# 4ment/physher

Hardware: AMD Instinct MI355X
Metric: lnL+gradient evals/sec, 1000-taxon GTR+G4 fp64, 1e6 site patterns (higher is better)
Workload: dtype f64

## Files before the change

include/physher_amd.h:

```cpp
#ifndef PHYSHER_AMD_H
#define PHYSHER_AMD_H

#include <stddef.h>
#include <stdint.h>

#ifdef __cplusplus
extern "C" {
#endif

typedef struct phyamd_engine phyamd_engine;

enum {
	PHYAMD_OK = 0,
	PHYAMD_EINVAL = -1,
	PHYAMD_EDEVICE = -2,
	PHYAMD_ENOMEM = -3,
	PHYAMD_EUNSUPPORTED = -4
};

enum { PHYAMD_RESCALE_NEVER = 0, PHYAMD_RESCALE_ALWAYS = 1, PHYAMD_RESCALE_AUTO = 2 };

enum {
	PHYAMD_GRAD_FOLD_ROOT_FREQS = 1,
	PHYAMD_GRAD_COMPAT_SCALED = 2
// ... 99 lines not shown
int phyamd_get_site_lnl_profile(phyamd_engine *e, phyamd_site_lnl_profile *out);
int phyamd_synchronize(phyamd_engine *e);

int phyamd_get_pattern_log_likelihoods(phyamd_engine *e, double *out );
int phyamd_get_partials(phyamd_engine *e, int node, int upper, double *out);
int phyamd_get_node_matrices(phyamd_engine *e, int node, int derivative, double *out );
int phyamd_post_order_parks(int32_t tip_count, const int32_t *left , const int32_t *right, int32_t root, int32_t second_slot,
                            int32_t *out , int32_t capacity);
#define PHYAMD_PRE_ORDER_COLUMNS 30
int phyamd_pre_order_schedule(int32_t tip_count, const int32_t *left , const int32_t *right, int32_t root, int32_t form,
                              int32_t *out , int32_t capacity, int32_t *hbm_slots);
int phyamd_post_order_slots(int32_t tip_count, const int32_t *left , const int32_t *right, int32_t root,
                            int32_t *out , int32_t capacity, int32_t *slots);
int phyamd_stream_elisions(int32_t tip_count, const int32_t *left , const int32_t *right, int32_t root,
                           int32_t *out , int32_t capacity);
int phyamd_is_rescaling(phyamd_engine *e);
int phyamd_set_rescaling(phyamd_engine *e, int policy);
int phyamd_set_keep_partials(phyamd_engine *e, int on);

typedef struct {
	double matrices_ms, lower_ms, upper_ms, reduce_ms;
	int32_t lower_launches, upper_launches;
	int64_t device_bytes;
	int32_t tiles;
} phyamd_profile;
int phyamd_set_reduction_levels(phyamd_engine *e, int levels);
int phyamd_set_profiling(phyamd_engine *e, int on);
int phyamd_get_profile(phyamd_engine *e, phyamd_profile *out);

#ifdef __cplusplus
// ... 4 lines not shown
```

physher_amd/_lib.py:

```python
from __future__ import annotations

import ctypes as C
import os

_HERE = os.path.dirname(os.path.abspath(__file__))
LIB_PATH = os.environ.get("PHYAMD_LIB") or os.path.join(_HERE, "libphysher_amd.so")

ABI_VERSION = 5

OK, EINVAL, EDEVICE, ENOMEM, EUNSUPPORTED = 0, -1, -2, -3, -4
RESCALE_NEVER, RESCALE_ALWAYS, RESCALE_AUTO = 0, 1, 2
GRAD_FOLD_ROOT_FREQS, GRAD_COMPAT_SCALED = 1, 2


class Config(C.Structure):
    _fields_ = [
        ("tip_count", C.c_int32), ("pattern_count", C.c_int32), ("state_count", C.c_int32),
        ("category_count", C.c_int32), ("device", C.c_int32), ("rescale", C.c_int32),
        ("max_device_bytes", C.c_int64), ("stream", C.c_void_p),
    ]


class Profile(C.Structure):
    _fields_ = [
# ... 91 lines not shown
    ("phyamd_branch_hessian", C.c_int, [_P, C.c_int, _P, _P, _P]),
    ("phyamd_get_hessian_profile", C.c_int, [_P, C.POINTER(HessianProfile)]),
    ("phyamd_get_general_profile", C.c_int, [_P, C.POINTER(GeneralProfile)]),
    ("phyamd_gradient_batch_weights", C.c_int, [_P, C.c_int, C.c_int32, _P, _P, _P, _P]),
    ("phyamd_get_weight_batch_profile", C.c_int, [_P, C.POINTER(WeightBatchProfile)]),
    ("phyamd_pattern_log_likelihoods_trees", C.c_int, [_P, C.c_int, C.c_int32, _P, _P, _P, _P, _P, _P, C.c_int32, _P, _P]),
    ("phyamd_get_site_lnl_profile", C.c_int, [_P, C.POINTER(SiteLnlProfile)]),
    ("phyamd_synchronize", C.c_int, [_P]),
    ("phyamd_get_pattern_log_likelihoods", C.c_int, [_P, _P]),
    ("phyamd_get_partials", C.c_int, [_P, C.c_int, C.c_int, _P]),
    ("phyamd_get_node_matrices", C.c_int, [_P, C.c_int, C.c_int, _P]),
    ("phyamd_post_order_parks", C.c_int, [C.c_int32, _P, _P, C.c_int32, C.c_int32, _P, C.c_int32]),
    ("phyamd_post_order_slots", C.c_int, [C.c_int32, _P, _P, C.c_int32, _P, C.c_int32, _P]),
    ("phyamd_pre_order_schedule", C.c_int, [C.c_int32, _P, _P, C.c_int32, C.c_int32, _P, C.c_int32, _P]),
    ("phyamd_stream_elisions", C.c_int, [C.c_int32, _P, _P, C.c_int32, _P, C.c_int32]),
    ("phyamd_is_rescaling", C.c_int, [_P]),
    ("phyamd_set_rescaling", C.c_int, [_P, C.c_int]),
    ("phyamd_set_keep_partials", C.c_int, [_P, C.c_int]),
    ("phyamd_set_reduction_levels", C.c_int, [_P, C.c_int]),
    ("phyamd_set_profiling", C.c_int, [_P, C.c_int]),
    ("phyamd_get_profile", C.c_int, [_P, C.POINTER(Profile)]),
    ("phyamd_store", C.c_int, [_P]),
    ("phyamd_restore", C.c_int, [_P]),
    ("phyamd_compress_patterns", C.c_int, [C.c_int, C.c_int32, C.c_int64, _P, _P, C.POINTER(C.c_int32), _P, _P]),
]

_lib = None


def load():
# ... 21 lines not shown
```

physher_amd/csrc/phyamd_abi.inc:

```

#include <condition_variable>
#include <functional>
#include <mutex>
#include <thread>

namespace {

class ShardWorkers {
public:
	explicit ShardWorkers(int n) : done_(0), generation_(0), stop_(false) {
		for (int i = 0; i < n; i++) threads_.emplace_back([this, i] { loop(i); });
	}
	~ShardWorkers() {
		{
			std::lock_guard<std::mutex> lk(m_);
			stop_ = true;
			generation_++;
		}
		cv_.notify_all();
		for (auto &t : threads_) t.join();
	}
	void run(const std::function<void(int)> &fn) {
		std::unique_lock<std::mutex> lk(m_);
		fn_ = &fn;
// ... 854 lines not shown
	if (!left || !right) return fail(PHYAMD_EINVAL, "null left or right");
	if (capacity < 0 || (capacity > 0 && !out)) return fail(PHYAMD_EINVAL, "null out with capacity %d", capacity);
	Schedule sched;
	StreamTables stream_tab;
	const std::string err = build_schedule(TreeRef{tip_count, left, right, root}, ScheduleOptions{}, &sched);
	if (!err.empty()) return fail(PHYAMD_EINVAL, "%s", err.c_str());
	build_stream_tables(sched, StreamGeometry{1, 1, WAVE, true}, &stream_tab);
	const std::vector<StreamElision> &el = stream_tab.elisions;
	for (int i = 0; i < (int)el.size() && i < capacity; i++) {
		const int32_t rec[8] = {el[i].node, el[i].parent, el[i].stored, el[i].sibling, el[i].sibling_kind, el[i].source, el[i].side, el[i].chunk};
		std::memcpy(out + (size_t)i * 8, rec, sizeof(rec));
	}
	return (int)el.size();
}

int phyamd_is_rescaling(phyamd_engine *g) {
	CHECK_GROUP(g);
	int any = 0;
	for (Shard *s : g->shards) any |= shard_is_rescaling(s);
	return any;
}

int phyamd_get_profile(phyamd_engine *g, phyamd_profile *out) {
	CHECK_GROUP(g);
	if (!out) return fail(PHYAMD_EINVAL, "null out");
	int rc;
	if ((rc = shard_get_profile(g->shards[0], out))) return rc;
	for (int i = 1; i < group_size(g); i++) {
		phyamd_profile p;
		if ((rc = shard_get_profile(g->shards[i], &p))) return rc;
// ... 12 lines not shown
```

physher_amd/csrc/phyamd_launch.inc:

```

size_t gen_image_doubles(const Shard *e) {
	return e->S == 20 ? MatImage<2, 5>::SIZE : e->S == 60 ? MatImage<4, 15>::SIZE : MatImage<4, 16>::SIZE;
}

template <int RT, int KT>
void launch_matrix_images(Shard *e, int count, const double *src, double *dst, const double *rowscale) {
	hipLaunchKernelGGL((k_matrix_images<RT, KT>), dim3(count), dim3(256), 0, e->stream, e->S, src, dst, rowscale);
}

void build_matrix_images(Shard *e, int count, const double *src, double *dst, const double *rowscale = nullptr) {
	if (e->S == 20) launch_matrix_images<2, 5>(e, count, src, dst, rowscale);
	else if (e->S == 60) launch_matrix_images<4, 15>(e, count, src, dst, rowscale);
	else launch_matrix_images<4, 16>(e, count, src, dst, rowscale);
}

int update_matrices(Shard *e) {
	if (e->generic && e->state.qimg_dirty && e->have_Q && e->have_freqs) {
		build_matrix_images(e, 1, e->d_Q, e->d_imgs + (size_t)e->N * e->C * gen_image_doubles(e));
		build_matrix_images(e, 1, e->d_Q, e->d_imgs + ((size_t)e->N * e->C + 1) * gen_image_doubles(e), e->d_freqs);
		HIP_TRY(hipGetLastError());
		q_images_rebuilt(e);
	}
	if (!e->state.matrices_dirty) return PHYAMD_OK;
	if (e->have_eigen) {
// ... 379 lines not shown
int launch_upper_stream(Shard *e) {
	int rc;
	const int nb = (e->P + WAVE - 1) / WAVE, R = e->stream_tab.R, nops = (int)e->stream_tab.ops.size();
	if ((size_t)nb * e->C * R > (size_t)e->N * e->C * e->gpart_row) return fail(PHYAMD_EDEVICE, "gradient slab too small for the streamed walk");
	e->d_gslab = e->d_gpart;
	if (e->stream_tab.P != e->P || e->stream_tab.mstride != e->mstride) {
		if ((rc = upload_schedule(e))) return rc;
		if (e->stream_tab.P != e->P || e->stream_tab.mstride != e->mstride) return fail(PHYAMD_EDEVICE, "streamed walk: descriptors do not match the pattern storage");
	}
	if ((rc = e->d_oct.ensure((size_t)8 * e->C * R))) return rc;
	const StreamVariant v = stream_variant(e->lower_form, SCALE);
	if (v.scale < 0) return fail(PHYAMD_EDEVICE, "streamed walk: the stored lowers hold the %s form, which no %s post-order pass writes", form_name(e->lower_form), SCALE ? "rescaled" : "plain");
	const bool exp2 = v.scale == 2, tf = v.tf;
	if (exp2 && (rc = e->d_uexp.ensure(std::max<size_t>(1, upper_slots_held(e)) * e->C * e->P))) return rc;
	const int waves = SCALE && !exp2 ? e->C : STREAM_WAVES;
	const size_t lds = (size_t)STREAM_LDS_PER_WAVE * waves + (exp2 ? (size_t)waves * STREAM_PARK_SLOTS * WAVE * sizeof(int) : SCALE ? (size_t)4 * e->C * WAVE * sizeof(double) : 0);
	const dim3 grid_x(SCALE && !exp2 ? (unsigned)nb : (unsigned)((nb + STREAM_WAVES - 1) / STREAM_WAVES) * e->C), block(WAVE, waves);
	hipLaunchKernelGGL(k_op_tables, dim3(nops, e->C), dim3(64), 0, e->stream, nops, e->C, (const int *)e->d_stream_op_tips, (const int *)e->d_stream_op_deep,
	                   (const int *)e->d_stream_site_tab, e->d_mats, FOLD ? e->d_Q : e->d_Qpi, reinterpret_cast<double *>(e->d_optab.get()));
	const int subtrees = (int)e->sched.walk_chunk_off.size() - 2;
	for (int phase = 0; phase < (subtrees > 0 ? 2 : 1); phase++) {
		const bool amb = e->stream_ambiguous;
		auto *kernel = exp2 ? (amb ? k_upper4_stream<FOLD, 2, true, true> : k_upper4_stream<FOLD, 2, false, true>)
		             : SCALE ? (amb ? k_upper4_stream<FOLD, 1, true, false> : k_upper4_stream<FOLD, 1, false, false>)
		             : tf    ? (amb ? k_upper4_stream<FOLD, 0, true, true> : k_upper4_stream<FOLD, 0, false, true>)
		                     : (amb ? k_upper4_stream<FOLD, 0, true, false> : k_upper4_stream<FOLD, 0, false, false>);
		const bool plain = !tf && !e->stream_tab.plain_desc.empty();
		hipLaunchKernelGGL(kernel, dim3(grid_x.x, phase ? subtrees : 1), block, lds, e->stream,
		                   (const StreamDesc *)e->d_stream_ops + (plain ? e->stream_tab.desc.size() : 0), (const StreamChunk *)e->d_stream_chunks + (plain ? e->stream_tab.chunks.size() : 0),
		                   (const int *)e->d_walk_chunk_off, phase, nops, e->P, e->C, nb, (const uint32_t *)e->d_mstream, e->mstride, (const double *)e->d_lower, e->d_upper,
		                   (const double *)e->d_mats, (const char *)e->d_optab, (const double *)(FOLD ? e->d_Q : e->d_Qpi), (const double *)e->d_freqs, (const double *)e->d_wl,
// ... 417 lines not shown
```

physher_amd/csrc/phyamd_schedule.inc:

```

int bind_device(Shard *e) {
	HIP_TRY(hipSetDevice(e->device));
	return PHYAMD_OK;
}

size_t node_partial_doubles(const Shard *e) { return (size_t)e->C * e->S * (e->generic ? e->Pp : e->P); }
size_t lower_slots(const Shard *e) { return e->d_lower.size() / node_partial_doubles(e); }
size_t upper_slots_held(const Shard *e) { return e->d_upper.size() / node_partial_doubles(e); }

int ensure_lower_storage(Shard *e) {
	const size_t need = (size_t)std::max(1, e->sched.core_count) * (e->two_slots ? 2 : 1);
	if (lower_slots(e) >= need) return PHYAMD_OK;
	e->d_lower.release();
	e->d_lscale.release();
	return e->d_lower.ensure(need * node_partial_doubles(e));
}

void refresh_op_cores(Schedule &s) {
	for (std::vector<NodeOp> *ops : {&s.lower_ops, &s.upper_ops, &s.walk_lower_ops, &s.walk_upper_ops, &s.walk_chunk_ops, &s.walk_lower_chunk_ops})
		for (NodeOp &op : *ops) {
			op.core_parent = s.core_index[op.parent];
			op.core_left = s.core_index[op.left];
			op.core_right = s.core_index[op.right];
		}
// ... 9 lines not shown
		HIP_TRY(hipMemcpyAsync(e->d_tiptab + (size_t)e->T * e->C * 64, e->sched.deep_host.data(), e->sched.deep_host.size() * sizeof(DeepDesc), hipMemcpyHostToDevice,
		                       e->stream));
	if (e->sched.walking || e->sched.gen_walking) {
		if ((rc = e->d_walk_lower_ops.ensure(e->N)) || (rc = e->d_walk_upper_ops.ensure(e->N))) return rc;
		HIP_TRY(hipMemcpyAsync(e->d_walk_lower_ops, e->sched.walk_lower_ops.data(), e->sched.walk_lower_ops.size() * sizeof(NodeOp), hipMemcpyHostToDevice, e->stream));
		HIP_TRY(hipMemcpyAsync(e->d_walk_upper_ops, e->sched.walk_upper_ops.data(), e->sched.walk_upper_ops.size() * sizeof(NodeOp), hipMemcpyHostToDevice, e->stream));
	}
	if (e->sched.walking) {
		if ((rc = e->d_walk_chunk_ops.ensure(e->N)) || (rc = e->d_walk_chunk_off.ensure((size_t)e->N + 2))) return rc;
		HIP_TRY(hipMemcpyAsync(e->d_walk_chunk_ops, e->sched.walk_chunk_ops.data(), e->sched.walk_chunk_ops.size() * sizeof(NodeOp), hipMemcpyHostToDevice, e->stream));
		HIP_TRY(hipMemcpyAsync(e->d_walk_chunk_off, e->sched.walk_chunk_off.data(), e->sched.walk_chunk_off.size() * sizeof(int), hipMemcpyHostToDevice, e->stream));
		if ((rc = e->d_walk_lower_chunk_ops.ensure(e->N)) || (rc = e->d_walk_lower_chunk_off.ensure((size_t)e->N + 2))) return rc;
		HIP_TRY(hipMemcpyAsync(e->d_walk_lower_chunk_ops, e->sched.walk_lower_chunk_ops.data(), e->sched.walk_lower_chunk_ops.size() * sizeof(NodeOp), hipMemcpyHostToDevice, e->stream));
		HIP_TRY(hipMemcpyAsync(e->d_walk_lower_chunk_off, e->sched.walk_lower_chunk_off.data(), e->sched.walk_lower_chunk_off.size() * sizeof(int), hipMemcpyHostToDevice, e->stream));
		if (stream_possible(e)) {
			build_stream_tables(e->sched, StreamGeometry{e->P, e->C, (size_t)e->nblk_walk_upper * e->G * WAVE, e->stream_elide_on}, &e->stream_tab);
			if ((rc = e->d_stream_ops.ensure((size_t)2 * e->N)) || (rc = e->d_stream_chunks.ensure((size_t)2 * e->N + 4)) ||
			    (rc = e->d_stream_row_entries.ensure(std::max((size_t)e->N * 32, e->stream_tab.row_entries.size()))) ||
			    (rc = e->d_stream_site_tab.ensure((size_t)e->N * 16)) || (rc = e->d_stream_qnode.ensure(e->N)) || (rc = e->d_stream_op_tips.ensure((size_t)e->N * 12)) ||
			    (rc = e->d_stream_flag.ensure(1)) || (rc = e->d_stream_op_deep.ensure(e->N)))
				return rc;
			HIP_TRY(hipMemcpyAsync(e->d_stream_op_tips, e->stream_tab.op_tips.data(), e->stream_tab.op_tips.size() * sizeof(int), hipMemcpyHostToDevice, e->stream));
			HIP_TRY(hipMemcpyAsync(e->d_stream_op_deep, e->stream_tab.op_deep.data(), e->stream_tab.op_deep.size() * sizeof(int), hipMemcpyHostToDevice, e->stream));
			HIP_TRY(hipMemcpyAsync(e->d_stream_ops, e->stream_tab.desc.data(), e->stream_tab.desc.size() * sizeof(StreamDesc), hipMemcpyHostToDevice, e->stream));
			HIP_TRY(hipMemcpyAsync(e->d_stream_chunks, e->stream_tab.chunks.data(), e->stream_tab.chunks.size() * sizeof(StreamChunk), hipMemcpyHostToDevice, e->stream));
			if (!e->stream_tab.plain_desc.empty()) {
				HIP_TRY(hipMemcpyAsync(e->d_stream_ops + e->stream_tab.desc.size(), e->stream_tab.plain_desc.data(), e->stream_tab.plain_desc.size() * sizeof(StreamDesc),
				                       hipMemcpyHostToDevice, e->stream));
				HIP_TRY(hipMemcpyAsync(e->d_stream_chunks + e->stream_tab.chunks.size(), e->stream_tab.plain_chunks.data(),
				                       e->stream_tab.plain_chunks.size() * sizeof(StreamChunk), hipMemcpyHostToDevice, e->stream));
			}
// ... 42 lines not shown
```

physher_amd/csrc/phyamd_shard.inc:

```

enum class LowerForm { Reference, Carried, CarriedExp2 };

struct ScheduleCounts { int core_count, upper_slots, widest; };

struct Shard {
	phyamd_config cfg{};
	DeviceBudget mem;
	DeviceBudget tile_mem{&mem};
	int T = 0, N = 0, P = 0, S = 0, C = 0, root = -1;
	int G = 1;
	bool generic = false;
	int Pp = 0;
	int nblk_root = 0;
	int nblk_lower = 0;
	int nblk_walk = 0, nblk_walk_upper = 0;
	int lower_walk_slots[2] = {0, 0};
	int gen_slots[3][2] = {};
	int lnl_blocks = 0;
	int grad_blocks = 0;
	size_t gpart_row = 0;
	struct State {
		bool all_dirty = true;
		std::vector<int> changed;
		bool force_root = false;
// ... 67 lines not shown
	int device = 0;
	hipStream_t stream = nullptr;
	bool own_stream = false;

	std::vector<int32_t> left, right;
	std::vector<double> lengths, model, freqs, rates, props;
	std::vector<double> lengths_sent;
	std::vector<uint8_t> explicit_host;
	bool have_topology = false, have_lengths = false, have_eigen = false, have_freqs = false, have_rates = false, have_weights = false;
	std::vector<uint8_t> tip_set;
	bool scaling_on = false;
	LowerForm lower_form = LowerForm::Reference;
	bool reference_form_only = false;
	bool exp2_on = true, tform_on = true;
	bool lower_park2_on = true;
	bool stream_elide_on = true;
	DeviceArray<int> d_lexp{&tile_mem}, d_uexp{&tile_mem}, d_Ec{&tile_mem}, d_Eroot{&tile_mem};
	bool keep_partials = false;
	bool profiling = false;
	bool prof_pending = false, prof_with_upper = false;

	Schedule sched;
	Schedule sched_spare;
	StreamTables stream_tab;
	ScheduleCounts scaled_counts{0, 0, 1};
	bool have_scaled_counts = false;
	bool fusion_enabled = true;

	DeviceArray<uint8_t> d_tipmask{&tile_mem};
	DeviceArray<unsigned long long> d_tipsets{&mem};
// ... 243 lines not shown
```

physher_amd/csrc/phyamd_shard_api.inc:

```

ScheduleCounts schedule_counts(const Schedule &s) {
	ScheduleCounts c{s.core_count, std::max(s.upper_slots, s.walk_upper_slots), 1};
	for (size_t i = 0; i + 1 < s.lower_level_off.size(); i++) c.widest = std::max(c.widest, s.lower_level_off[i + 1] - s.lower_level_off[i]);
	for (size_t i = 0; i + 1 < s.upper_level_off.size(); i++) c.widest = std::max(c.widest, s.upper_level_off[i + 1] - s.upper_level_off[i]);
	return c;
}

double tile_working_set(const Shard *e, double p, bool exact, const ScheduleCounts &k) {
	const double pp = e->S == 4 ? p : std::ceil(p / 16.0) * 16.0, npd = (double)e->C * e->S * pp;
	const double per_pattern = (double)e->T * p + 8.0 * p * (3.0 + (e->S == 4 ? 0.0 : (double)e->C));
	const bool may_scale = e->cfg.rescale != PHYAMD_RESCALE_NEVER, exponents = may_scale && e->S == 4 && e->exp2_on;
	if (!exact) return 8.0 * (exponents ? 1.125 : 1.0) * ((e->S == 4 ? 0.5 : 1.6) * (double)(e->N - e->T) * npd + 2.0 * npd) + per_pattern;
	double doubles = (double)(std::max(1, k.core_count) + std::max(1, k.upper_slots)) * npd;
	if (may_scale) doubles += (double)std::max(1, k.core_count) * p + (e->S == 4 ? 0.0 : 5.0 * k.widest * e->C * p);
	if (exponents) doubles += 0.5 * ((double)(std::max(1, k.core_count) + std::max(1, k.upper_slots) + 1) * e->C * p + p);
	if (e->S == 4) doubles += (double)e->C * p;
	doubles += (double)e->N * e->C * (p / (WAVE * std::max(1, 4 / e->C)) + 1.0);
	if (e->S == 4) doubles += 2.0 * e->N * (p / (WAVE * PPT_UPPER) + 19.0) + 0.5 * p / 64.0;
	return 8.0 * doubles + per_pattern;
}

double tile_working_set(const Shard *e, double p, bool exact) {
	const double now = tile_working_set(e, p, exact, schedule_counts(e->sched));
	return e->have_scaled_counts ? std::max(now, tile_working_set(e, p, exact, e->scaled_counts)) : now;
// ... 136 lines not shown
	if (cfg->stream) e->stream = (hipStream_t)cfg->stream;
	else {
		hipError_t err = hipStreamCreateWithFlags(&e->stream, hipStreamNonBlocking);
		if (err != hipSuccess) return bail(fail(PHYAMD_EDEVICE, "hipStreamCreate: %s", hipGetErrorString(err)));
		e->own_stream = true;
	}
	e->scaling_on = cfg->rescale == PHYAMD_RESCALE_ALWAYS;
	if (const char *env = std::getenv("PHYAMD_FUSE")) e->fusion_enabled = std::atoi(env) != 0;
	if (const char *env = std::getenv("PHYAMD_WALK")) e->walk_enabled = std::atoi(env) != 0;
	if (const char *env = std::getenv("PHYAMD_GEN_FUSION")) e->generic_fusion = std::atoi(env) != 0;
	if (const char *env = std::getenv("PHYAMD_XCD_MAP")) e->xcd_map = std::atoi(env) != 0;
	if (const char *env = std::getenv("PHYAMD_SCALE_EXP2")) e->exp2_on = std::atoi(env) != 0;
	if (const char *env = std::getenv("PHYAMD_STREAM_TFORM")) e->tform_on = std::atoi(env) != 0;
	if (const char *env = std::getenv("PHYAMD_LOWER_PARK2")) e->lower_park2_on = std::atoi(env) != 0;
	if (const char *env = std::getenv("PHYAMD_STREAM_ELIDE")) e->stream_elide_on = std::atoi(env) != 0;
	e->generic = e->S != 4;
	e->tip_set.assign(e->T, 0);
	e->tip_empty.assign(e->T, 0);
	e->mem.spare = &e->batch_mem;
	e->batch_max_patterns = BATCH_MAX_PATTERNS;
	if (const char *env = std::getenv("PHYAMD_BATCH_MAX_PATTERNS")) e->batch_max_patterns = std::atoi(env);
	if (const char *env = std::getenv("PHYAMD_BATCH_TRACE")) e->batch_trace = std::atoi(env) != 0;
	e->explicit_host.assign(e->N, 0);
	const size_t msz = (size_t)e->N * e->C * e->S * e->S;
	if (e->generic && ((rc = e->d_tipsets.ensure(256)) || (rc = e->d_imgs.ensure(((size_t)e->N * e->C + 2) * gen_image_doubles(e))))) return bail(rc);
	if (e->S == 20 && GenFuse<2>::QP) {
		if ((rc = e->d_qp_mats.ensure((size_t)e->T * e->C * e->S * e->S)) || (rc = e->d_qp_imgs.ensure((size_t)e->T * e->C * gen_image_doubles(e)))) return bail(rc);
	}
	if ((rc = e->d_mats.ensure(msz)) || (rc = e->d_dmats.ensure(msz)) || (rc = e->d_model.ensure((size_t)e->S + 2 * e->S * e->S)) ||
	    (rc = e->d_Q.ensure((size_t)e->S * e->S)))
// ... 895 lines not shown
```

physher_amd/csrc/phyamd_tree_schedule.h:

```cpp
#ifndef PHYAMD_TREE_SCHEDULE_H
#define PHYAMD_TREE_SCHEDULE_H

#include <algorithm>
#include <cstdarg>
#include <cstdint>
#include <cstdio>
#include <string>
#include <utility>
#include <vector>

#include "phyamd_types.h"

struct TreeRef {
	int T;
	const int32_t *left, *right;
	int root;
};

inline std::string schedule_error(const char *fmt, ...) {
	char buf[512];
	va_list ap;
	va_start(ap, fmt);
	vsnprintf(buf, sizeof buf, fmt, ap);
	va_end(ap);
// ... 526 lines not shown
		sc.walk_upper_ops.reserve(tree.T - 1);
		b.walk_post_order();
		b.walk_pre_order();
		if (sc.walking) {
			chunk_pre_order(sc);
			chunk_post_order(sc);
		}
	}
	return std::string();
}

struct StreamGeometry {
	int P, C;
	size_t mstride;
	bool elide = false;
};

struct StreamElision {
	int32_t node, parent, stored, sibling, sibling_kind;
	int32_t source;
	int32_t side;
	int32_t chunk;
};

struct StreamTables {
	std::vector<StreamOp> ops;
	std::vector<StreamDesc> desc;
	int P = 0;
	size_t mstride = 0;
	std::vector<StreamChunk> chunks;
	std::vector<LowerDesc> lower_desc;
	std::vector<LowerChunk> lower_chunks;
	std::vector<int> row_entries;
	std::vector<int> site_tab;
	std::vector<int> qnode;
	std::vector<int> op_tips;
	std::vector<int> op_deep;
	std::vector<StreamDesc> plain_desc;
	std::vector<StreamChunk> plain_chunks;
	std::vector<StreamElision> elisions;
	int words = 0, R = 0;
};

struct MaskPacker {
	std::vector<int> &rows;
	int row = -1, used = 32, entries = 8;
	explicit MaskPacker(std::vector<int> &r) : rows(r), row((int)r.size() / 8 - 1) {}
	void add(const int *tips, int &out_row, int &out_shift) {
		int span = 0, n = 0;
		for (int j = 0; j < 6; j++)
			if (tips[j] >= 0) {
				span = j + 1;
				n++;
			}
		const int bits = 1 + 4 * span;
// ... 374 lines not shown
			ch.mask_words = words;
			ch.same_row = same_row;
			if (want[0] >= 0) ch.a = want[0];
			if (want[1] >= 0) ch.b = want[1];
		} else {
			StreamDesc &pv = t.desc[i - 1];
			pv.flags = (pv.flags & ~(3 << 14 | 1 << 24 | 1 << 25)) | words << 14 | two_pieces << 24 | same_row << 25;
			pv.nx_words = (int64_t)first_word * row_bytes;
			if (want[0] >= 0) pv.nx_a = (int64_t)want[0] * array_bytes;
			if (want[1] >= 0) pv.nx_b = (int64_t)want[1] * array_bytes;
		}
	}
	t.words = (int)t.row_entries.size() / 8;
}

inline void build_stream_tables(const Schedule &sc, const StreamGeometry &g, StreamTables *out) {
	stream_pre_order(sc, g, *out);
	stream_post_order(sc, g, *out);
	out->plain_desc.clear();
	out->plain_chunks.clear();
	out->elisions.clear();
	if (g.elide) stream_elide(sc, g, *out);
}


inline int build_batch_ops(int T, const int32_t *left, const int32_t *right, int root, std::vector<BatchOp> *ops, bool park_all = false) {
	const int N = 2 * T - 1;
	std::vector<int> size(N, 1), order;
	{
		std::vector<int> stack{root};
		while (!stack.empty()) {
			const int n = stack.back();
			stack.pop_back();
			order.push_back(n);
			if (n >= T) {
				stack.push_back(left[n]);
				stack.push_back(right[n]);
// ... 99 lines not shown
```

physher_amd/csrc/phyamd_types.h:

```cpp
#ifndef PHYAMD_TYPES_H
#define PHYAMD_TYPES_H

#include <cstddef>
#include <cstdint>

constexpr int WAVE = 64;

enum { CH_TIP = 0, CH_CORE = 1, CH_DEEP = 2, CH_CHERRY = 3, CH_CHERRY_TIP = 4 };

struct DeepDesc {
	int32_t kind_left, left, lt0, lt1, lt2, linner;
	int32_t kind_right, right, rt0, rt1, rt2, rinner;
};

struct NodeOp {
	int32_t parent;
	int32_t left, right;
	int32_t upper_slot_parent;
	int32_t upper_slot_left, upper_slot_right;
	int32_t core_parent, core_left, core_right;
	int32_t kind_left, kind_right;
	int32_t lt0, lt1, lt2, linner;
	int32_t rt0, rt1, rt2, rinner;
	int32_t carry_in;
// ... 24 lines not shown
	int32_t lnode, la[10];
	int32_t rnode, ra[10];
	int32_t nx_u;
	int32_t wsh;
};
static_assert(sizeof(StreamOp) == 128, "one StreamOp = 32 dwords");

struct StreamDesc {
	int32_t flags;
	int32_t parent, lnode, rnode;
	int32_t lm[5], rm[5];
	int64_t nx_words;
	int64_t nx_a, nx_b, nx_u;
	int64_t st_left, st_right;
	int32_t wsh;
	int32_t pad[5];
};
static_assert(sizeof(StreamDesc) == 128 && offsetof(StreamDesc, nx_words) == 56, "one StreamDesc = 32 dwords");

struct StreamChunk {
	int32_t mask_word, mask_words, a, b, u, same_row, pad[2];
};

constexpr int OPBLK_BYTES = 2048, OPBLK_LEFT = 64, OPBLK_RIGHT = 1024, OPTIP_BYTES = 160;

constexpr int STREAM_PARK_SLOTS = 2;

struct LowerDesc {
	int32_t flags;
	int32_t nx_block;
	int32_t lnode, rnode, lm[5], rm[5];
	int64_t nx_words;
	int64_t store;
	int64_t mem_l, mem_r;
	int32_t wsh;
	int32_t self;
	int64_t ls_store, ls_l, ls_r;
	int32_t pad[2];
};
static_assert(sizeof(LowerDesc) == 128 && offsetof(LowerDesc, nx_words) == 56, "one LowerDesc = 32 dwords");
struct LowerChunk {
// ... 6 lines not shown
```

physher_amd/csrc/phyamd_walk4s.inc:

```


__global__ __launch_bounds__(256) void k_build_mask_stream(int rows, int P, size_t mstride, const int *__restrict__ row_entries, const uint8_t *__restrict__ tipmask,
                                                           uint32_t *__restrict__ mstream, int *__restrict__ flags) {
	const size_t k = (size_t)blockIdx.x * 256 + threadIdx.x;
	if (k >= mstride) return;
	bool bad = false, amb = false;
	for (int w = blockIdx.y; w < rows; w += gridDim.y) {
		uint32_t v = 0;
		for (int j = 0; j < 8; j++) {
			const int ent = row_entries[w * 8 + j];
			if (ent < 0) continue;
			const int t = ent & 0xFFFFF, pos = (ent >> 20) & 31, fpos = (ent >> 25) & 31;
			const uint32_t m = (k < (size_t)P ? tipmask[(size_t)t * P + k] : 0xFu) & 0xFu;
			const uint32_t code = m == 1 ? 0 : m == 2 ? 1 : m == 4 ? 2 : m == 8 ? 3 : (m == 15 || m == 0) ? 4 : m == 3 ? 5 : m < 8 ? m + 1 : m;
			bad |= m == 0;
			if (code >= 5) {
				amb = true;
				v |= 1u << fpos;
			}
			v |= code << pos;
		}
		mstream[(size_t)w * mstride + k] = v;
	}
	if (bad || amb) atomicOr(flags, (bad ? 1 : 0) | (amb ? 2 : 0));
// ... 197 lines not shown

typedef double dv4 __attribute__((ext_vector_type(4)));
__device__ __forceinline__ d4 prefetch4(const char *base, unsigned lane_off, bool nt) {
	dv2 lo, hi;
	if (nt) asm volatile("global_load_dwordx4 %0, %2, %3 nt\n\tglobal_load_dwordx4 %1, %2, %3 offset:16 nt" : "=&v"(lo), "=&v"(hi) : "v"(lane_off), "s"(base) : "memory");
	else asm volatile("global_load_dwordx4 %0, %2, %3\n\tglobal_load_dwordx4 %1, %2, %3 offset:16" : "=&v"(lo), "=&v"(hi) : "v"(lane_off), "s"(base) : "memory");
	return d4{lo.x, lo.y, hi.x, hi.y};
}
__device__ __forceinline__ unsigned prefetch1(const char *base, unsigned lane_off) {
	unsigned w;
	asm volatile("global_load_dword %0, %1, %2" : "=v"(w) : "v"(lane_off), "s"(base) : "memory");
	return w;
}

constexpr int STREAM_PARK_BYTES = 2 * WAVE * 16;
constexpr int STREAM_LDS_PER_WAVE = STREAM_PARK_SLOTS * STREAM_PARK_BYTES + 2 * OPBLK_BYTES;

constexpr int STREAM_WAVES = 4;

__device__ __forceinline__ unsigned xcd_position(unsigned x, unsigned n, int on) {
	if (!on) return x;
	const unsigned r = x & 7u, q = n >> 3, m = n & 7u;
	return r * q + (r < m ? r : m) + (x >> 3);
}

__device__ __forceinline__ void any_value(d4 &v) { asm volatile("" : "=v"(v.x), "=v"(v.y), "=v"(v.z), "=v"(v.w)); }
__device__ __forceinline__ d4 own_registers(const d4 &v) {
	d4 r;
	asm volatile("v_mov_b64 %0, %1" : "=v"(r.x) : "v"(v.x));
	asm volatile("v_mov_b64 %0, %1" : "=v"(r.y) : "v"(v.y));
	asm volatile("v_mov_b64 %0, %1" : "=v"(r.z) : "v"(v.z));
	asm volatile("v_mov_b64 %0, %1" : "=v"(r.w) : "v"(v.w));
	return r;
}
template <bool FOLD, int SCALE, bool AMBIG = false, bool TF = false>
__global__ __launch_bounds__(STREAM_WAVES *WAVE, (SCALE || AMBIG) ? STREAM_MIN_WAVES_SCALE : STREAM_MIN_WAVES) void k_upper4_stream(
    const StreamDesc *__restrict__ ops, const StreamChunk *__restrict__ chunks, const int *__restrict__ chunk_off, int chunk_base, int nops, int P, int C, int nb,
    const uint32_t *__restrict__ mstream, size_t mstride, const double *__restrict__ lower, double *__restrict__ upper, const double *__restrict__ mats,
    const char *__restrict__ optab, const double *__restrict__ Q, const double *__restrict__ freqs, const double *__restrict__ w_over_L,
    double *__restrict__ gslab, int R, const double *__restrict__ props, const double *__restrict__ weights, int xcd_map, const int *__restrict__ lexp,
    int *__restrict__ uexp, const int *__restrict__ Eroot) {
	extern __shared__ double sh[];
	constexpr bool KEEP_BN = !SCALE && !AMBIG;
	constexpr bool XCH = SCALE == 1, EXP2 = SCALE == 2;
	const int lane = threadIdx.x, wv = __builtin_amdgcn_readfirstlane(threadIdx.y);
	const unsigned vx = XCH ? blockIdx.x : xcd_position(blockIdx.x, gridDim.x, xcd_map);
	const int c = XCH ? wv : vx % C, blk = XCH ? (int)blockIdx.x : (int)(vx / C) * STREAM_WAVES + wv;
	if (blk >= nb) return;
	const size_t plane = (size_t)P * 4;
	const int k0 = blk * WAVE + lane;
	const bool valid = k0 < P;
	const unsigned k = valid ? k0 : P - 1;
	const unsigned poff = k * 32u;
	const unsigned moff = (unsigned)k0 * 4u;
	const lds_cptr wave_lds = (lds_cptr)sh + (size_t)wv * STREAM_LDS_PER_WAVE;
	const lds_cptr blocks = wave_lds + STREAM_PARK_SLOTS * STREAM_PARK_BYTES;
	SX x{reinterpret_cast<const char *>(mats + (size_t)c * 16), blocks};
	const double wl = SCALE ? 1.0 : (valid ? w_over_L[k] : 0.0);
	const double wk = XCH ? (valid ? weights[k] : 0.0) : EXP2 ? (valid ? w_over_L[k] : 0.0) : 0.0;
	const double pc = XCH ? props[c] : 0.0;
	const int eroot = EXP2 ? Eroot[k] : 0;
	double *const xbase = sh + (size_t)blockDim.y * (STREAM_LDS_PER_WAVE / 8);
	const int xsz = blockDim.y * WAVE;
	int *const pexp = reinterpret_cast<int *>(xbase) + ((size_t)wv * STREAM_PARK_SLOTS) * WAVE + lane;
	const char *const lexp_c = EXP2 ? reinterpret_cast<const char *>(lexp) + (size_t)c * P * 4 : nullptr;
	char *const uexp_c = EXP2 ? reinterpret_cast<char *>(uexp) + (size_t)c * P * 4 : nullptr;
	const unsigned eoff = k * 4u;
	SiteSum<SCALE != 0> ss;
	ss.Q = as_const(Q);
	ss.sel0 = (lane & 3) == 0 ? 1.0 : 0.0;
	ss.sel1 = (lane & 3) == 1 ? 1.0 : 0.0;
// ... 9 lines not shown

	const char *const lower_c = reinterpret_cast<const char *>(lower + (size_t)c * plane);
	char *const upper_c = reinterpret_cast<char *>(upper + (size_t)c * plane);
	const char *const mstream_b = reinterpret_cast<const char *>(mstream);
	const size_t mrow = mstride * 4;
	constexpr bool ASM_PREFETCH = true;
	auto lower_at = [&](int64_t off) -> d4 {
		return ASM_PREFETCH ? prefetch4(lower_c + off, poff, true) : load4_stream(reinterpret_cast<const double *>(lower_c + off + poff));
	};
	auto upper_at = [&](int64_t off) -> d4 { return ASM_PREFETCH ? prefetch4(upper_c + off, poff, false) : load4(reinterpret_cast<const double *>(upper_c + off + poff)); };
	auto store_upper_at = [&](int64_t off, const d4 &v) { store4(reinterpret_cast<double *>(upper_c + off + poff), v); };
	auto word_at = [&](int64_t off) -> unsigned { return ASM_PREFETCH ? prefetch1(mstream_b + off, moff) : *reinterpret_cast<const unsigned *>(mstream_b + off + moff); };
	auto fetch_lower = [&](int core) -> d4 { return load4_stream(reinterpret_cast<const double *>(reinterpret_cast<const char *>(lower + ((size_t)core * C + c) * plane) + poff)); };
	auto fetch_upper = [&](int slot) -> d4 { return load4(reinterpret_cast<const double *>(reinterpret_cast<const char *>(upper + ((size_t)slot * C + c) * plane) + poff)); };
	auto fetch_word = [&](int w) -> unsigned { return *reinterpret_cast<const unsigned *>(reinterpret_cast<const char *>(mstream + (size_t)w * mstride) + moff); };
	auto fetch_block = [&](int op_index, bool two) {
		const char *src = optab_c + (size_t)op_index * OPBLK_BYTES;
		const lds_cptr dst = blocks + (op_index & 1) * OPBLK_BYTES;
		dma_piece(src, dst);
		if (two) dma_piece(src + 1024, dst + 1024);
	};

	unsigned w0 = 0, w1 = 0;
	d4 A = d4{1., 1., 1., 1.}, B = A, U = A;
	int eA = 0, eB = 0, eU = 0;
	if (op_begin < op_end) {
		const StreamChunk ch = chunks[chunk];
		fetch_block(op_begin, true);
		if (ch.mask_words > 0) w0 = fetch_word(ch.mask_word);
		if (ch.mask_words > 1) w1 = fetch_word(ch.mask_word + (ch.same_row ? 0 : 1));
// ... 6 lines not shown
			if (ch.u != -1) eU = *reinterpret_cast<const int *>(uexp_c + (size_t)ch.u * C * P * 4 + eoff);
		}
	}
	d4 ul = A;
	int e_ul = 0;
	double prev_tot = 0.0;
	int prev_off = -1;
#pragma unroll 1
	for (int i = op_begin; i < op_end; i++) {
		StreamDesc op;
		{
			typedef const __attribute__((address_space(4))) int32_t *ciptr;
			const ciptr raw = (ciptr)(ops + i);
			int32_t *dst = reinterpret_cast<int32_t *>(&op);
#pragma unroll
			for (int j = 0; j < 27; j++) dst[j] = raw[j];
		}
		asm volatile("s_waitcnt vmcnt(0)" ::: "memory");
		if (prev_off >= 0) *reinterpret_cast<double *>(slab + (unsigned)prev_off) = prev_tot;
		const int fl = op.flags;
		const int kl = fl & 7, kr = (fl >> 3) & 7;
		const int usrc = (fl >> 9) & 7, pk = (fl >> 12) & 3, nxw = (fl >> 14) & 3;
		x.tb = blocks + (i & 1) * OPBLK_BYTES;
		const int soff = *(const __attribute__((address_space(3))) int *)(x.tb + cid4);
		const unsigned g0 = w0 >> (op.wsh & 31), g1 = w1 >> ((op.wsh >> 5) & 31);
		const unsigned wL = g0, wR = (kl != CH_CORE) ? g1 : g0;
		if (AMBIG) x.amb = __any((int)((g0 | (kl != CH_CORE && kr != CH_CORE ? g1 : 0u)) & 1u)) != 0;
		d4 a;
		int ea = 0;
		if (usrc == SU_CARRY) {
			a = matvec4_opt<false>(x.M(op.parent), ul);
// ... 2 lines not shown
			const int ps = STREAM_PARK_SLOTS > 1 ? ((fl >> 7) & 1) * (STREAM_PARK_BYTES / 16) : 0;
			const dv2 lo = park[ps], hi = park[ps + WAVE];
			a = matvec4_opt<false>(x.M(op.parent), d4{lo.x, lo.y, hi.x, hi.y});
			if (EXP2) ea = pexp[(STREAM_PARK_SLOTS > 1 ? (fl >> 7) & 1 : 0) * WAVE];
		} else if (usrc == SU_U) {
			ea = eU;
			a = matvec4_opt<false>(x.M(op.parent), U);
			if (!SCALE && !valid) a = d4{0., 0., 0., 0.};
		}
		else a = FOLD ? d4{wl * freqs[0], wl * freqs[1], wl * freqs[2], wl * freqs[3]} : d4{wl, wl, wl, wl};
		d4 bl, br, bnl, bnr;
		if (KEEP_BN) {
			any_value(bnl);
			any_value(bnr);
		}
		if (kl == CH_CORE) bl = TF ? own_registers(A) : matvec4_opt<false>(x.M(op.lnode), A);
		else if (kl == CH_TIP) bl = x.site_tip<0, 0>(wL);
		else if (kl == CH_DEEP)
			bl = matvec4_opt<false>(x.M(op.lnode), mul4(s_half<0, 0>(x, (fl >> 16) & 3, op.lm[0], op.lm[1], wL), s_half<0, 3>(x, (fl >> 18) & 3, op.lm[2], op.lm[3], wL)));
		else if (TF && kl >= SK_CORE_TIP) bl = s_elided_message<0>(x, kl, op.lnode, op.lm[0], wL, A);
		else bl = s_fringe_message<0, KEEP_BN>(x, kl, op.lnode, op.lm[4], wL, bnl);
		if (kr == CH_CORE) br = TF ? own_registers(B) : matvec4_opt<false>(x.M(op.rnode), B);
		else if (kr == CH_TIP) br = x.site_tip<1, 0>(wR);
		else if (kr == CH_DEEP)
			br = matvec4_opt<false>(x.M(op.rnode), mul4(s_half<1, 0>(x, (fl >> 20) & 3, op.rm[0], op.rm[1], wR), s_half<1, 3>(x, (fl >> 22) & 3, op.rm[2], op.rm[3], wR)));
		else if (TF && kr >= SK_CORE_TIP) br = s_elided_message<1>(x, kr, op.rnode, op.rm[0], wR, B);
		else br = s_fringe_message<1, KEEP_BN>(x, kr, op.rnode, op.rm[4], wR, bnr);
		const int e_bl = EXP2 && (kl == CH_CORE || kl >= SK_CORE_TIP) ? eA : 0, e_br = EXP2 && (kr == CH_CORE || kr >= SK_CORE_TIP) ? eB : 0;
		__builtin_amdgcn_s_setprio(3);
		unsigned nw0 = 0, nw1 = 0;
		if (i + 1 < op_end) fetch_block(i + 1, (fl >> 24) & 1);
		if (nxw > 0) nw0 = word_at(op.nx_words);
		if (nxw > 1) nw1 = word_at(op.nx_words + ((fl >> 25) & 1 ? (int64_t)0 : (int64_t)mrow));
		if (fl & (1 << 26)) A = lower_at(op.nx_a);
		if (fl & (1 << 27)) B = lower_at(op.nx_b);
		if (fl & (1 << 28)) U = upper_at(op.nx_u);
		if (EXP2) {
			if (fl & (1 << 26)) eA = *reinterpret_cast<const int *>(lexp_c + (op.nx_a >> 3) + eoff);
			if (fl & (1 << 27)) eB = *reinterpret_cast<const int *>(lexp_c + (op.nx_b >> 3) + eoff);
			if (fl & (1 << 28)) eU = *reinterpret_cast<const int *>(uexp_c + (op.nx_u >> 3) + eoff);
		}
// ... 290 lines not shown
```

Measured before the change: 37.84.

## Hand off deep-child half messages via LDS to the next stream op

```diff
diff --git a/include/physher_amd.h b/include/physher_amd.h
--- a/include/physher_amd.h
+++ b/include/physher_amd.h
@@ -137,6 +137,8 @@
                             int32_t *out , int32_t capacity, int32_t *slots);
 int phyamd_stream_elisions(int32_t tip_count, const int32_t *left , const int32_t *right, int32_t root,
                            int32_t *out , int32_t capacity);
+int phyamd_stream_handoffs(int32_t tip_count, const int32_t *left , const int32_t *right, int32_t root, int32_t areas,
+                           int32_t *out , int32_t capacity);
 int phyamd_is_rescaling(phyamd_engine *e);
 int phyamd_set_rescaling(phyamd_engine *e, int policy);
 int phyamd_set_keep_partials(phyamd_engine *e, int on);
diff --git a/physher_amd/_lib.py b/physher_amd/_lib.py
--- a/physher_amd/_lib.py
+++ b/physher_amd/_lib.py
@@ -129,6 +129,7 @@
     ("phyamd_post_order_slots", C.c_int, [C.c_int32, _P, _P, C.c_int32, _P, C.c_int32, _P]),
     ("phyamd_pre_order_schedule", C.c_int, [C.c_int32, _P, _P, C.c_int32, C.c_int32, _P, C.c_int32, _P]),
     ("phyamd_stream_elisions", C.c_int, [C.c_int32, _P, _P, C.c_int32, _P, C.c_int32]),
+    ("phyamd_stream_handoffs", C.c_int, [C.c_int32, _P, _P, C.c_int32, C.c_int32, _P, C.c_int32]),
     ("phyamd_is_rescaling", C.c_int, [_P]),
     ("phyamd_set_rescaling", C.c_int, [_P, C.c_int]),
     ("phyamd_set_keep_partials", C.c_int, [_P, C.c_int]),
diff --git a/physher_amd/csrc/phyamd_abi.inc b/physher_amd/csrc/phyamd_abi.inc
--- a/physher_amd/csrc/phyamd_abi.inc
+++ b/physher_amd/csrc/phyamd_abi.inc
@@ -892,6 +892,24 @@
 	return (int)el.size();
 }
 
+int phyamd_stream_handoffs(int32_t tip_count, const int32_t *left, const int32_t *right, int32_t root, int32_t areas, int32_t *out, int32_t capacity) {
+	if (tip_count < 2) return fail(PHYAMD_EINVAL, "tip_count must be >= 2 (got %d)", tip_count);
+	if (!left || !right) return fail(PHYAMD_EINVAL, "null left or right");
+	if (areas > 1) return fail(PHYAMD_EINVAL, "areas must be 0, 1 or negative (got %d)", areas);
+	if (capacity < 0 || (capacity > 0 && !out)) return fail(PHYAMD_EINVAL, "null out with capacity %d", capacity);
+	Schedule sched;
+	StreamTables stream_tab;
+	const std::string err = build_schedule(TreeRef{tip_count, left, right, root}, ScheduleOptions{}, &sched);
+	if (!err.empty()) return fail(PHYAMD_EINVAL, "%s", err.c_str());
+	build_stream_tables(sched, StreamGeometry{1, 1, WAVE, true, true, areas < 0 ? STREAM_HANDOFF_AREAS : areas}, &stream_tab);
+	const std::vector<StreamHandoff> &hd = stream_tab.handoffs;
+	for (int i = 0; i < (int)hd.size() && i < capacity; i++) {
+		const int32_t rec[8] = {hd[i].parent, hd[i].node, hd[i].half, hd[i].place, hd[i].chunk, hd[i].kind, hd[i].own_side, hd[i].op};
+		std::memcpy(out + (size_t)i * 8, rec, sizeof(rec));
+	}
+	return (int)hd.size();
+}
+
 int phyamd_is_rescaling(phyamd_engine *g) {
 	CHECK_GROUP(g);
 	int any = 0;
diff --git a/physher_amd/csrc/phyamd_launch.inc b/physher_amd/csrc/phyamd_launch.inc
--- a/physher_amd/csrc/phyamd_launch.inc
+++ b/physher_amd/csrc/phyamd_launch.inc
@@ -417,7 +417,8 @@
 	const bool exp2 = v.scale == 2, tf = v.tf;
 	if (exp2 && (rc = e->d_uexp.ensure(std::max<size_t>(1, upper_slots_held(e)) * e->C * e->P))) return rc;
 	const int waves = SCALE && !exp2 ? e->C : STREAM_WAVES;
-	const size_t lds = (size_t)STREAM_LDS_PER_WAVE * waves + (exp2 ? (size_t)waves * STREAM_PARK_SLOTS * WAVE * sizeof(int) : SCALE ? (size_t)4 * e->C * WAVE * sizeof(double) : 0);
+	const size_t lds = (size_t)stream_lds_per_wave(stream_handoff_areas(v.scale, e->stream_ambiguous, tf)) * waves +
+	                   (exp2 ? (size_t)waves * STREAM_PARK_SLOTS * WAVE * sizeof(int) : SCALE ? (size_t)4 * e->C * WAVE * sizeof(double) : 0);
 	const dim3 grid_x(SCALE && !exp2 ? (unsigned)nb : (unsigned)((nb + STREAM_WAVES - 1) / STREAM_WAVES) * e->C), block(WAVE, waves);
 	hipLaunchKernelGGL(k_op_tables, dim3(nops, e->C), dim3(64), 0, e->stream, nops, e->C, (const int *)e->d_stream_op_tips, (const int *)e->d_stream_op_deep,
 	                   (const int *)e->d_stream_site_tab, e->d_mats, FOLD ? e->d_Q : e->d_Qpi, reinterpret_cast<double *>(e->d_optab.get()));
diff --git a/physher_amd/csrc/phyamd_schedule.inc b/physher_amd/csrc/phyamd_schedule.inc
--- a/physher_amd/csrc/phyamd_schedule.inc
+++ b/physher_amd/csrc/phyamd_schedule.inc
@@ -47,7 +47,8 @@
 		HIP_TRY(hipMemcpyAsync(e->d_walk_lower_chunk_ops, e->sched.walk_lower_chunk_ops.data(), e->sched.walk_lower_chunk_ops.size() * sizeof(NodeOp), hipMemcpyHostToDevice, e->stream));
 		HIP_TRY(hipMemcpyAsync(e->d_walk_lower_chunk_off, e->sched.walk_lower_chunk_off.data(), e->sched.walk_lower_chunk_off.size() * sizeof(int), hipMemcpyHostToDevice, e->stream));
 		if (stream_possible(e)) {
-			build_stream_tables(e->sched, StreamGeometry{e->P, e->C, (size_t)e->nblk_walk_upper * e->G * WAVE, e->stream_elide_on}, &e->stream_tab);
+			build_stream_tables(e->sched, StreamGeometry{e->P, e->C, (size_t)e->nblk_walk_upper * e->G * WAVE, e->stream_elide_on, e->stream_handoff_on, STREAM_HANDOFF_AREAS},
+			                    &e->stream_tab);
 			if ((rc = e->d_stream_ops.ensure((size_t)2 * e->N)) || (rc = e->d_stream_chunks.ensure((size_t)2 * e->N + 4)) ||
 			    (rc = e->d_stream_row_entries.ensure(std::max((size_t)e->N * 32, e->stream_tab.row_entries.size()))) ||
 			    (rc = e->d_stream_site_tab.ensure((size_t)e->N * 16)) || (rc = e->d_stream_qnode.ensure(e->N)) || (rc = e->d_stream_op_tips.ensure((size_t)e->N * 12)) ||
diff --git a/physher_amd/csrc/phyamd_shard.inc b/physher_amd/csrc/phyamd_shard.inc
--- a/physher_amd/csrc/phyamd_shard.inc
+++ b/physher_amd/csrc/phyamd_shard.inc
@@ -105,6 +105,7 @@
 	bool reference_form_only = false;
 	bool exp2_on = true, tform_on = true;
 	bool lower_park2_on = true;
+	bool stream_handoff_on = true;
 	bool stream_elide_on = true;
 	DeviceArray<int> d_lexp{&tile_mem}, d_uexp{&tile_mem}, d_Ec{&tile_mem}, d_Eroot{&tile_mem};
 	bool keep_partials = false;
diff --git a/physher_amd/csrc/phyamd_shard_api.inc b/physher_amd/csrc/phyamd_shard_api.inc
--- a/physher_amd/csrc/phyamd_shard_api.inc
+++ b/physher_amd/csrc/phyamd_shard_api.inc
@@ -174,6 +174,7 @@
 	if (const char *env = std::getenv("PHYAMD_STREAM_TFORM")) e->tform_on = std::atoi(env) != 0;
 	if (const char *env = std::getenv("PHYAMD_LOWER_PARK2")) e->lower_park2_on = std::atoi(env) != 0;
 	if (const char *env = std::getenv("PHYAMD_STREAM_ELIDE")) e->stream_elide_on = std::atoi(env) != 0;
+	if (const char *env = std::getenv("PHYAMD_STREAM_HANDOFF")) e->stream_handoff_on = std::atoi(env) != 0;
 	e->generic = e->S != 4;
 	e->tip_set.assign(e->T, 0);
 	e->tip_empty.assign(e->T, 0);
diff --git a/physher_amd/csrc/phyamd_tree_schedule.h b/physher_amd/csrc/phyamd_tree_schedule.h
--- a/physher_amd/csrc/phyamd_tree_schedule.h
+++ b/physher_amd/csrc/phyamd_tree_schedule.h
@@ -564,6 +564,17 @@
 	int P, C;
 	size_t mstride;
 	bool elide = false;
+	bool handoff = false;
+	int handoff_areas = 0;
+};
+
+struct StreamHandoff {
+	int32_t parent, node, half;
+	int32_t place;
+	int32_t chunk;
+	int32_t kind;
+	int32_t own_side;
+	int32_t op;
 };
 
 struct StreamElision {
@@ -589,6 +600,7 @@
 	std::vector<StreamDesc> plain_desc;
 	std::vector<StreamChunk> plain_chunks;
 	std::vector<StreamElision> elisions;
+	std::vector<StreamHandoff> handoffs;
 	int words = 0, R = 0;
 };
 
@@ -993,13 +1005,69 @@
 	t.words = (int)t.row_entries.size() / 8;
 }
 
+inline void stream_handoff(const Schedule &sc, const StreamGeometry &g, StreamTables &t) {
+	t.handoffs.clear();
+	const int ns = (int)t.ops.size();
+	for (int k = 0; k + 1 < (int)sc.walk_chunk_off.size(); k++) {
+		bool busy[2] = {false, false};
+		for (int i = sc.walk_chunk_off[k]; i < sc.walk_chunk_off[k + 1] && i < ns; i++) {
+			const StreamOp &s = t.ops[i];
+			const int fl = t.desc[i].flags, usrc = (fl >> 9) & 7, pk = (fl >> 12) & 3;
+			if (usrc == SU_LDS) busy[(fl >> 7) & 1] = false;
+			if (i + 1 < sc.walk_chunk_off[k + 1]) {
+				const StreamOp &own = t.ops[i + 1];
+				const int ofl = t.desc[i + 1].flags, ousrc = (ofl >> 9) & 7, opk = (ofl >> 12) & 3;
+				for (int side = 0; side < 2; side++) {
+					if (((fl >> (3 * side)) & 7) != CH_DEEP || (side ? s.rnode : s.lnode) != own.parent) continue;
+					bool taken[2] = {false, false};
+					int areas = g.handoff_areas;
+					for (int h = 0; h < 2; h++) {
+						const int hk = (fl >> (16 + 4 * side + 2 * h)) & 3;
+						if (hk == HK_TIP) continue;
+						const int half_node = (side ? s.ra : s.la)[5 * h];
+						const int own_side = own.lnode == half_node ? 0 : 1;
+						if ((own_side ? own.rnode : own.lnode) != half_node) continue;
+						const int own_kind = (ofl >> (3 * own_side)) & 7;
+						if (own_kind != (hk == HK_CHERRY ? (int)CH_CHERRY : (int)CH_CHERRY_TIP)) continue;
+						int place = HAND_NONE;
+						if (areas > 0) {
+							place = HAND_AREA;
+							areas--;
+						} else
+							for (int sl = 0; sl < STREAM_PARK_SLOTS && sl < 2 && place == HAND_NONE; sl++) {
+								const bool parent_parks = pk && ((fl >> 6) & 1) == sl;
+								const bool own_touches = (ousrc == SU_LDS && ((ofl >> 7) & 1) == sl) || (opk && ((ofl >> 6) & 1) == sl);
+								if (!busy[sl] && !taken[sl] && !parent_parks && !own_touches) {
+									place = sl == 0 ? HAND_SLOT0 : HAND_SLOT1;
+									taken[sl] = true;
+								}
+							}
+						if (place == HAND_NONE) continue;
+						const int32_t write = place << (4 * side + 2 * h), take = place << (8 + 2 * own_side);
+						t.desc[i].hand |= write;
+						t.desc[i + 1].hand |= take;
+						if (!t.plain_desc.empty()) {
+							t.plain_desc[i].hand |= write;
+							t.plain_desc[i + 1].hand |= take;
+						}
+						t.handoffs.push_back(StreamHandoff{s.parent, own.parent, h, place, k, hk == HK_CHERRY ? (int)CH_CHERRY : (int)CH_CHERRY_TIP, own_side, i});
+					}
+				}
+			}
+			if (pk) busy[(fl >> 6) & 1] = true;
+		}
+	}
+}
+
 inline void build_stream_tables(const Schedule &sc, const StreamGeometry &g, StreamTables *out) {
 	stream_pre_order(sc, g, *out);
 	stream_post_order(sc, g, *out);
 	out->plain_desc.clear();
 	out->plain_chunks.clear();
 	out->elisions.clear();
+	out->handoffs.clear();
 	if (g.elide) stream_elide(sc, g, *out);
+	if (g.handoff) stream_handoff(sc, g, *out);
 }
 
 
diff --git a/physher_amd/csrc/phyamd_types.h b/physher_amd/csrc/phyamd_types.h
--- a/physher_amd/csrc/phyamd_types.h
+++ b/physher_amd/csrc/phyamd_types.h
@@ -62,7 +62,8 @@
 	int64_t nx_a, nx_b, nx_u;
 	int64_t st_left, st_right;
 	int32_t wsh;
-	int32_t pad[5];
+	int32_t hand;
+	int32_t pad[4];
 };
 static_assert(sizeof(StreamDesc) == 128 && offsetof(StreamDesc, nx_words) == 56, "one StreamDesc = 32 dwords");
 
@@ -73,6 +74,8 @@
 constexpr int OPBLK_BYTES = 2048, OPBLK_LEFT = 64, OPBLK_RIGHT = 1024, OPTIP_BYTES = 160;
 
 constexpr int STREAM_PARK_SLOTS = 2;
+constexpr int STREAM_HANDOFF_AREAS = 1;
+enum { HAND_NONE = 0, HAND_SLOT0 = 1, HAND_SLOT1 = 2, HAND_AREA = 3 };
 
 struct LowerDesc {
 	int32_t flags;
diff --git a/physher_amd/csrc/phyamd_walk4s.inc b/physher_amd/csrc/phyamd_walk4s.inc
--- a/physher_amd/csrc/phyamd_walk4s.inc
+++ b/physher_amd/csrc/phyamd_walk4s.inc
@@ -235,7 +235,9 @@
 }
 
 constexpr int STREAM_PARK_BYTES = 2 * WAVE * 16;
-constexpr int STREAM_LDS_PER_WAVE = STREAM_PARK_SLOTS * STREAM_PARK_BYTES + 2 * OPBLK_BYTES;
+constexpr bool stream_takes_handoffs(int scale, bool ambig, bool tf) { return true; }
+constexpr int stream_handoff_areas(int scale, bool ambig, bool tf) { return stream_takes_handoffs(scale, ambig, tf) && !(scale == 2 && !ambig) ? STREAM_HANDOFF_AREAS : 0; }
+constexpr int stream_lds_per_wave(int areas) { return (STREAM_PARK_SLOTS + areas) * STREAM_PARK_BYTES + 2 * OPBLK_BYTES; }
 
 constexpr int STREAM_WAVES = 4;
 
@@ -264,6 +266,8 @@
 	extern __shared__ double sh[];
 	constexpr bool KEEP_BN = !SCALE && !AMBIG;
 	constexpr bool XCH = SCALE == 1, EXP2 = SCALE == 2;
+	constexpr bool HAND = stream_takes_handoffs(SCALE, AMBIG, TF);
+	constexpr int AREAS = stream_handoff_areas(SCALE, AMBIG, TF), STREAM_LDS_PER_WAVE = stream_lds_per_wave(AREAS);
 	const int lane = threadIdx.x, wv = __builtin_amdgcn_readfirstlane(threadIdx.y);
 	const unsigned vx = XCH ? blockIdx.x : xcd_position(blockIdx.x, gridDim.x, xcd_map);
 	const int c = XCH ? wv : vx % C, blk = XCH ? (int)blockIdx.x : (int)(vx / C) * STREAM_WAVES + wv;
@@ -275,7 +279,7 @@
 	const unsigned poff = k * 32u;
 	const unsigned moff = (unsigned)k0 * 4u;
 	const lds_cptr wave_lds = (lds_cptr)sh + (size_t)wv * STREAM_LDS_PER_WAVE;
-	const lds_cptr blocks = wave_lds + STREAM_PARK_SLOTS * STREAM_PARK_BYTES;
+	const lds_cptr blocks = wave_lds + (STREAM_PARK_SLOTS + AREAS) * STREAM_PARK_BYTES;
 	SX x{reinterpret_cast<const char *>(mats + (size_t)c * 16), blocks};
 	const double wl = SCALE ? 1.0 : (valid ? w_over_L[k] : 0.0);
 	const double wk = XCH ? (valid ? weights[k] : 0.0) : EXP2 ? (valid ? w_over_L[k] : 0.0) : 0.0;
@@ -315,6 +319,16 @@
 	auto fetch_lower = [&](int core) -> d4 { return load4_stream(reinterpret_cast<const double *>(reinterpret_cast<const char *>(lower + ((size_t)core * C + c) * plane) + poff)); };
 	auto fetch_upper = [&](int slot) -> d4 { return load4(reinterpret_cast<const double *>(reinterpret_cast<const char *>(upper + ((size_t)slot * C + c) * plane) + poff)); };
 	auto fetch_word = [&](int w) -> unsigned { return *reinterpret_cast<const unsigned *>(reinterpret_cast<const char *>(mstream + (size_t)w * mstride) + moff); };
+	auto hand_put = [&](int place, const d4 &v) {
+		const int at = (place - 1) * (STREAM_PARK_BYTES / 16);
+		park[at] = dv2{v.x, v.y};
+		park[at + WAVE] = dv2{v.z, v.w};
+	};
+	auto hand_take = [&](int place) -> d4 {
+		const int at = (place - 1) * (STREAM_PARK_BYTES / 16);
+		const dv2 lo = park[at], hi = park[at + WAVE];
+		return d4{lo.x, lo.y, hi.x, hi.y};
+	};
 	auto fetch_block = [&](int op_index, bool two) {
 		const char *src = optab_c + (size_t)op_index * OPBLK_BYTES;
 		const lds_cptr dst = blocks + (op_index & 1) * OPBLK_BYTES;
@@ -351,7 +365,7 @@
 			const ciptr raw = (ciptr)(ops + i);
 			int32_t *dst = reinterpret_cast<int32_t *>(&op);
 #pragma unroll
-			for (int j = 0; j < 27; j++) dst[j] = raw[j];
+			for (int j = 0; j < (HAND ? 28 : 27); j++) dst[j] = raw[j];
 		}
 		asm volatile("s_waitcnt vmcnt(0)" ::: "memory");
 		if (prev_off >= 0) *reinterpret_cast<double *>(slab + (unsigned)prev_off) = prev_tot;
@@ -384,17 +398,31 @@
 			any_value(bnl);
 			any_value(bnr);
 		}
-		if (kl == CH_CORE) bl = TF ? own_registers(A) : matvec4_opt<false>(x.M(op.lnode), A);
+		const int hd = HAND ? op.hand : 0;
+		auto handed = [&](int place) { return HAND && place != HAND_NONE && (AREAS > 0 || place != HAND_AREA); };
+		if (handed((hd >> 8) & 3)) {
+			bl = hand_take((hd >> 8) & 3);
+			if (KEEP_BN && kl == CH_CHERRY_TIP) bnl = matvec4_opt<false>(x.M(op.lm[4]), mul4(x.site_tip<0, 0>(wL), x.site_tip<0, 1>(wL)));
+		} else if (kl == CH_CORE) bl = TF ? own_registers(A) : matvec4_opt<false>(x.M(op.lnode), A);
 		else if (kl == CH_TIP) bl = x.site_tip<0, 0>(wL);
-		else if (kl == CH_DEEP)
-			bl = matvec4_opt<false>(x.M(op.lnode), mul4(s_half<0, 0>(x, (fl >> 16) & 3, op.lm[0], op.lm[1], wL), s_half<0, 3>(x, (fl >> 18) & 3, op.lm[2], op.lm[3], wL)));
-		else if (TF && kl >= SK_CORE_TIP) bl = s_elided_message<0>(x, kl, op.lnode, op.lm[0], wL, A);
+		else if (kl == CH_DEEP) {
+			const d4 h0 = s_half<0, 0>(x, (fl >> 16) & 3, op.lm[0], op.lm[1], wL), h1 = s_half<0, 3>(x, (fl >> 18) & 3, op.lm[2], op.lm[3], wL);
+			if (handed(hd & 3)) hand_put(hd & 3, h0);
+			if (handed((hd >> 2) & 3)) hand_put((hd >> 2) & 3, h1);
+			bl = matvec4_opt<false>(x.M(op.lnode), mul4(h0, h1));
+		} else if (TF && kl >= SK_CORE_TIP) bl = s_elided_message<0>(x, kl, op.lnode, op.lm[0], wL, A);
 		else bl = s_fringe_message<0, KEEP_BN>(x, kl, op.lnode, op.lm[4], wL, bnl);
-		if (kr == CH_CORE) br = TF ? own_registers(B) : matvec4_opt<false>(x.M(op.rnode), B);
+		if (handed((hd >> 10) & 3)) {
+			br = hand_take((hd >> 10) & 3);
+			if (KEEP_BN && kr == CH_CHERRY_TIP) bnr = matvec4_opt<false>(x.M(op.rm[4]), mul4(x.site_tip<1, 0>(wR), x.site_tip<1, 1>(wR)));
+		} else if (kr == CH_CORE) br = TF ? own_registers(B) : matvec4_opt<false>(x.M(op.rnode), B);
 		else if (kr == CH_TIP) br = x.site_tip<1, 0>(wR);
-		else if (kr == CH_DEEP)
-			br = matvec4_opt<false>(x.M(op.rnode), mul4(s_half<1, 0>(x, (fl >> 20) & 3, op.rm[0], op.rm[1], wR), s_half<1, 3>(x, (fl >> 22) & 3, op.rm[2], op.rm[3], wR)));
-		else if (TF && kr >= SK_CORE_TIP) br = s_elided_message<1>(x, kr, op.rnode, op.rm[0], wR, B);
+		else if (kr == CH_DEEP) {
+			const d4 h0 = s_half<1, 0>(x, (fl >> 20) & 3, op.rm[0], op.rm[1], wR), h1 = s_half<1, 3>(x, (fl >> 22) & 3, op.rm[2], op.rm[3], wR);
+			if (handed((hd >> 4) & 3)) hand_put((hd >> 4) & 3, h0);
+			if (handed((hd >> 6) & 3)) hand_put((hd >> 6) & 3, h1);
+			br = matvec4_opt<false>(x.M(op.rnode), mul4(h0, h1));
+		} else if (TF && kr >= SK_CORE_TIP) br = s_elided_message<1>(x, kr, op.rnode, op.rm[0], wR, B);
 		else br = s_fringe_message<1, KEEP_BN>(x, kr, op.rnode, op.rm[4], wR, bnr);
 		const int e_bl = EXP2 && (kl == CH_CORE || kl >= SK_CORE_TIP) ? eA : 0, e_br = EXP2 && (kr == CH_CORE || kr >= SK_CORE_TIP) ? eB : 0;
 		__builtin_amdgcn_s_setprio(3);
```

Result: no change. 38.13, median of 6 (+0.8%).
